# uci-cbcl/esm-efficient

Hardware: AMD Instinct MI355X
Metric: residues/sec ESM2-650M fwd, 50k packed tokens; % bf16 MFMA peak; 1/2/4/8 GPU (higher is better)
Workload: dtype bf16

## Files before the change

### esm-efficient_amd/csrc/attn.hip

```cpp
#include "common.h"
#include "launch.h"
#include "gemm.h"

#include <atomic>
#include <type_traits>

namespace esme {

static constexpr int QT = 128;
static constexpr int KT = 64;
static constexpr int kAttnDma0 = 3, kAttnDma1 = 11;

struct AttnArgs {
    const u16* q; const u16* k; const u16* v; int64_t ld;
    u16* o; int64_t ldo;
    const int32_t* cu;
    int H;
    float scale_log2;
    int nqt;
    int nhb;
    float thr;
    int spec;
    const int32_t* order;
};

template <int D>
__device__ __forceinline__ int kswz(int row) {
    constexpr int CPR = D / 8;
    constexpr int RPB = 16 / CPR;
    return (row / RPB) & (CPR - 1);
}

template <int D, int QB, bool F16 = false>
__global__ __launch_bounds__(256, 2) void attn_varlen_kernel(const AttnArgs a) {
    constexpr int DS = D / 16;
    constexpr int DB = (D + 31) / 32;
    constexpr int CPR = D / 8;
    constexpr int KCH = KT * CPR;
    constexpr int KI = (KCH + 255) / 256;
    constexpr int DQ = D / 4;
    constexpr int DQ_HI_BITS = (D == 16 ? 0 : D == 32 ? 1 : D == 64 ? 2 : 3);
    constexpr int VI = (16 * DQ + 255) / 256;
    constexpr int K_BYTES = KT * D * 2;
    constexpr int BUF = K_BYTES + D * 128;
    const float THR = a.thr;

    __shared__ __attribute__((aligned(16))) char smem[2 * BUF];

    const int tid = threadIdx.x, lane = tid & 63, wave = tid >> 6;
    const int l31 = lane & 31, hi = lane >> 5;
    const int b = a.order ? a.order[blockIdx.z] : (int)blockIdx.z, h = blockIdx.y;
    const int s0 = a.cu[b], S = a.cu[b + 1] - s0;
    const int q0 = blockIdx.x * (QT * QB);
    if (q0 >= S) return;

    const unsigned int ld = (unsigned int)a.ld;
    const u16* qb = a.q + (int64_t)s0 * a.ld + h * D;
    const u16* kb = a.k + (int64_t)s0 * a.ld + h * D;
    const u16* vb = a.v + (int64_t)s0 * a.ld + h * D;

    int qrow[QB];
    bool blk_active[QB];
    bf16x8 qf[QB][DS];
#pragma unroll
    for (int b = 0; b < QB; ++b) {
        const int r0 = q0 + (wave * QB + b) * 32;
        qrow[b] = r0 + l31;
        blk_active[b] = r0 < S;
        const unsigned int qc = qrow[b] < S ? qrow[b] : S - 1;
#pragma unroll
        for (int ds = 0; ds < DS; ++ds)
            qf[b][ds] = *reinterpret_cast<const bf16x8*>(qb + (qc * ld + ds * 16 + hi * 8));
    }
    const bool wave_active = blk_active[0];

    unsigned int koff[KI];
    int krow[KI];
#pragma unroll
    for (int i = 0; i < KI; ++i) {
        const int c = i * 256 + tid;
        krow[i] = c / CPR;
        koff[i] = (unsigned int)(c % CPR) * 8u;
    }
    int v_dq[VI], v_kq[VI];
#pragma unroll
    for (int i = 0; i < VI; ++i) {
        const int rest = (lane >> 4) | (wave << 2) | (i << 4);
        v_dq[i] = (lane & 3) | ((rest & ((1 << DQ_HI_BITS) - 1)) << 2);
        v_kq[i] = ((lane >> 2) & 3) | ((rest >> DQ_HI_BITS) << 2);
    }
    u32x4 kreg[KI];
    u32x2 vreg[VI][4];
    auto load_tile = [&](int kv0) {
        const bool full = kv0 + KT <= S;
#pragma unroll
        for (int i = 0; i < KI; ++i) {
            if (KCH >= 256 * KI || krow[i] < KT) {
                unsigned int row = kv0 + krow[i];
                if (!full) row = row < (unsigned int)S ? row : S - 1;
                kreg[i] = *reinterpret_cast<const u32x4*>(kb + (row * ld + koff[i]));
            }
        }
#pragma unroll
        for (int i = 0; i < VI; ++i) {
            if (v_kq[i] < 16) {
#pragma unroll
// ... 388 lines not shown
#pragma unroll
                        for (int j = 0; j < 8; ++j) p[j] -= ph[j];
                        pf[NPT - 1][kbk][s] = __builtin_bit_cast(bf16x8, pack8t<F16>(p));
                    }
                }
            l_run += psum;

            const char* Vt = buf + 2 * K_BYTES;
#pragma unroll
            for (int i = 0; i < DB; ++i) {
                int drow = i * 32 + l31;
                if (D < 32) drow &= (D - 1);
                const char* rp = Vt + drow * 128;
                const int sw = (drow >> 1) & 7;
#pragma unroll
                for (int kbk = 0; kbk < 2; ++kbk)
#pragma unroll
                    for (int s = 0; s < 2; ++s) {
                        const bf16x8 vh = *reinterpret_cast<const bf16x8*>(rp + (((kbk * 4 + s * 2 + hi) ^ sw) << 4));
                        if constexpr (!QKP) {
                            ESME_LDS_CHECK(rp + V_BYTES + (((kbk * 4 + s * 2 + hi) ^ sw) << 4), 16, smem, 2 * BUF);
                            const bf16x8 vl = *reinterpret_cast<const bf16x8*>(rp + V_BYTES + (((kbk * 4 + s * 2 + hi) ^ sw) << 4));
                            oacc[i] = mfma_32x32x16<F16>(vl, pf[0][kbk][s], oacc[i]);
                            oacc[i] = mfma_32x32x16<F16>(vh, pf[NPT - 1][kbk][s], oacc[i]);
                        }
                        oacc[i] = mfma_32x32x16<F16>(vh, pf[0][kbk][s], oacc[i]);
                    }
            }
        }
        if (t + 1 < ntiles) {
            store_tile(smem + ((t + 1) & 1) * BUF);
            if (t + 2 < ntiles) load_tile(kv0 + 2 * KT);
        }
        __syncthreads();
    }

    if (!wave_active) return;
    const float l_tot = l_run + __shfl_xor(l_run, 32, 64);
    const float inv = 1.0f / l_tot;
    if (qrow < S) {
        u16* op = a.o + (int64_t)(s0 + qrow) * a.ldo + h * D;
#pragma unroll
        for (int i = 0; i < DB; ++i)
#pragma unroll
            for (int g = 0; g < 4; ++g) {
                const int d = i * 32 + 8 * g + 4 * hi;
                if (d < D) {
                    float o4[4];
#pragma unroll
                    for (int e = 0; e < 4; ++e) o4[e] = oacc[i][4 * g + e] * inv;
                    const u32x2 pk = {pack16<F16>(o4[0], o4[1]), pack16<F16>(o4[2], o4[3])};
                    *reinterpret_cast<u32x2*>(op + d) = pk;
                    if constexpr (!QKP) {
                        const u32x2 pl = {pack16<F16>(o4[0] - lo16<F16>(pk[0]), o4[1] - hi16<F16>(pk[0])), pack16<F16>(o4[2] - lo16<F16>(pk[1]), o4[3] - hi16<F16>(pk[1]))};
                        *reinterpret_cast<u32x2*>(op + sa.lo_out + d) = pl;
                    }
                }
            }
    }
}


template <int NW, bool QP = false, int D = 64, bool F16 = false>
__global__ __launch_bounds__(NW * 64, 2) void attn_pp64_kernel(const AttnArgs a) {
    constexpr float S0 = (QP && F16) ? -4.0f : 0.0f;
    constexpr int DS = D / 16, DB = D / 32, NT = NW * 64;
    constexpr int ROWB = D * 2;
    constexpr int K_BYTES = KT * D * 2;
    constexpr int SLOT = K_BYTES + D * 128;
    constexpr int ROWS = NW * 64;
    constexpr int NPV = 4 * DB, NQK = 2 * DS, NM = NPV + NQK;
    constexpr int PPS = 16 / NM;
    static_assert(D == 64 || D == 32, "head dims 64 and 32");
    static_assert(NW == 4 || (NW == 8 && D == 64), "4 waves (8: head dim 64 only)");
    extern __shared__ __attribute__((aligned(16))) char smem[];

    const int tid = threadIdx.x, lane = tid & 63;
    const int wave = __builtin_amdgcn_readfirstlane(tid >> 6);
    const int l31 = lane & 31, hi = lane >> 5;
    const unsigned int xcd = blockIdx.x & 7u, bi = blockIdx.x >> 3;
    const int qt = (int)(bi % (unsigned int)a.nqt);
    const unsigned int hb = (bi / (unsigned int)a.nqt) * 8u + xcd;
    if (hb >= (unsigned int)a.nhb) return;
    const int h = (int)(hb % (unsigned int)a.H), bi_seq = (int)(hb / (unsigned int)a.H);
    const int b = a.order ? a.order[bi_seq] : bi_seq;
    const int s0 = a.cu[b], S = a.cu[b + 1] - s0;
    const int q0 = qt * ROWS;
    if (q0 >= S) return;

    const unsigned int ld = (unsigned int)a.ld;
    const u16* qb = a.q + (int64_t)s0 * a.ld + h * D;
    const unsigned int kv_bytes = ((unsigned int)(S - 1) * ld + D) * 2u;
    auto make_rsrc = [&](const u16* p) -> u32x4 {
        const uint64_t v = (uint64_t)(uintptr_t)p;
        return u32x4{(unsigned int)__builtin_amdgcn_readfirstlane((int)(unsigned int)v),
                     (unsigned int)__builtin_amdgcn_readfirstlane((int)((unsigned int)(v >> 32) & 0xffffu)),
                     (unsigned int)__builtin_amdgcn_readfirstlane((int)kv_bytes), 0x00020000u};
    };
    const u32x4 krs = make_rsrc(a.k + (int64_t)s0 * a.ld + h * D);
    const u32x4 vrs = make_rsrc(a.v + (int64_t)s0 * a.ld + h * D);
    auto dma16 = [&](const u32x4 rs, const unsigned int voff, const char* dst) {
        ESME_LDS_CHECK(dst, 1024, smem, 4 * SLOT);
        const unsigned int d = (unsigned int)__builtin_amdgcn_readfirstlane((int)(unsigned int)(uintptr_t)dst);
        unsigned int keep;
        asm volatile("s_mov_b32 %0, m0\n\ts_mov_b32 m0, %2\n\ts_nop 0\n\tbuffer_load_dwordx4 %1, %3, 0 offen lds\n\ts_mov_b32 m0, %0"
                     : "=&s"(keep) : "v"(voff), "s"(d), "s"(rs) : "memory");
    };

    bf16x8 qf[2][DS];
    const int wrow0 = q0 + wave * 64;
    const bool wave_active = wrow0 < S;
#pragma unroll
    for (int bb = 0; bb < 2; ++bb) {
        const int qr = wrow0 + bb * 32 + l31;
        const unsigned int qc = qr < S ? qr : S - 1;
#pragma unroll
        for (int ds = 0; ds < DS; ++ds)
            qf[bb][ds] = *reinterpret_cast<const bf16x8*>(qb + (qc * ld + ds * 16 + hi * 8));
    }

    constexpr int KI = K_BYTES / (NW * 1024);
    constexpr int CPR = D / 8;
    const unsigned int tile_bytes = (unsigned int)KT * ld * 2u;
    unsigned int kg0, vg0;
    {
        const int r = wave * (64 / CPR) + lane / CPR, pch = lane % CPR;
        kg0 = ((unsigned int)r * ld + ((pch ^ kswz<D>(r)) * 8)) * 2u;
        vg0 = ((unsigned int)r * ld + ((D == 64 ? (pch ^ (((r >> 1) & 1) << 2)) : pch) * 8)) * 2u;
    }
    const unsigned int kg_step = (unsigned int)(NW * (64 / CPR)) * ld * 2u;
    auto dma_k = [&](int tile, char* slot) {
        const unsigned int base = (unsigned int)tile * tile_bytes + kg0;
#pragma unroll
        for (int i = 0; i < KI; ++i)
            dma16(krs, base + i * kg_step, slot + (i * NW + wave) * 1024);
    };
    auto dma_v = [&](int tile, char* slot) {
        const unsigned int base = (unsigned int)tile * tile_bytes + vg0;
#pragma unroll
        for (int i = 0; i < KI; ++i)
            dma16(vrs, base + i * kg_step, slot + K_BYTES + (i * NW + wave) * 1024);
    };

    const int krow_perm = (l31 & 3) | (((l31 >> 3) & 1) << 2) | (((l31 >> 2) & 1) << 3) | (l31 & 16);
    int kfo[DS];
#pragma unroll
    for (int i = 0; i < DS; ++i) kfo[i] = krow_perm * ROWB + (((i * 2 + hi) ^ kswz<D>(krow_perm)) << 4);
    int vb[DB];
    {
        const int j = (lane & 15) >> 2, p = lane & 3, gsel = (lane >> 4) & 1;
#pragma unroll
        for (int db = 0; db < DB; ++db) vb[db] = K_BYTES + (hi * 8 + j) * ROWB + (D == 64 ? ((db ^ (j >> 1)) * 64) : 0) + gsel * 32 + p * 8;
    }
    typedef short s16x4 __attribute__((ext_vector_type(4)));
    auto vfrag = [&](const char* Vs, const int db, const int ks) -> bf16x8 {
        typedef __attribute__((address_space(3))) s16x4* ltr_t;
        const char* p = Vs + vb[db] + ks * (16 * ROWB);
        ESME_LDS_CHECK(p, 8, smem, 4 * SLOT); ESME_LDS_CHECK(p + 4 * ROWB, 8, smem, 4 * SLOT);
        const s16x4 lo = __builtin_amdgcn_ds_read_tr16_b64_v4i16((ltr_t)(p));
        const s16x4 up = __builtin_amdgcn_ds_read_tr16_b64_v4i16((ltr_t)(p + 4 * ROWB));
        return __builtin_bit_cast(bf16x8, __builtin_shufflevector(lo, up, 0, 1, 2, 3, 4, 5, 6, 7));
    };

    f32x16 oacc[2][DB], sacc[2][2];
    u32x4 pw[2][2][2];
    float mc[2], lrun[2];
    const float c = a.scale_log2, thr = a.thr;
// ... 634 lines not shown
    static std::atomic<unsigned long long> done{0ull};
    if (const int rc = raise_dynamic_lds(done, kern, smem, "attn")) return rc;
    sa.a.nqt = (max_len + 127) / 128;
    const int64_t blocks = (int64_t)sa.a.nqt * (((int64_t)sa.a.H * B + 7) / 8) * 8;
    if (blocks > 0x7fffffffLL) return fail(ESME_ERR_UNSUPPORTED, "attn: grid too large");
    hipLaunchKernelGGL(kern, dim3((unsigned int)blocks), dim3(256), smem, s, sa);
    return check_launch("attn_varlen_fwd");
}

static constexpr int kMaxGridZ = 65535;

static int generic_launch_ok(int64_t ld_qkv, int max_len, int rows, int B, const int32_t* seq_order, const char* what) {
    if (((int64_t)max_len + rows) * ld_qkv >= (1LL << 32)) {
        snprintf(error_buffer(), kErrorBufferSize, "%s: (max_len + %d) * ld_qkv must stay below 2^32 elements (32-bit row offsets "
                 "inside one sequence)", what, rows);
        return ESME_ERR_UNSUPPORTED;
    }
    if (seq_order && B > kMaxGridZ) {
        snprintf(error_buffer(), kErrorBufferSize, "%s: seq_order is not supported with more than 65535 sequences", what);
        return ESME_ERR_ARG;
    }
    return ESME_OK;
}

static AttnArgs sequence_chunk(AttnArgs a, int b0, int nb) {
    a.cu += b0;
    a.nhb = a.H * nb;
    return a;
}

template <int D, int QB, bool F16>
static int launch_generic(const AttnArgs& a, int B, int max_len, hipStream_t s) {
    constexpr int rows = QT * QB;
    if (const int rc = generic_launch_ok(a.ld, max_len, rows, B, a.order, "attn")) return rc;
    return for_sequence_chunks(B, kMaxGridZ, [&](int b0, int nb) {
        const dim3 grid((unsigned int)((max_len + rows - 1) / rows), (unsigned int)a.H, (unsigned int)nb);
        hipLaunchKernelGGL((attn_varlen_kernel<D, QB, F16>), grid, dim3(256), 0, s, sequence_chunk(a, b0, nb));
        return check_launch("attn_varlen_fwd");
    });
}

template <int D, bool F16, bool QKP>
static int launch_split(const AttnSplitArgs& sa, int B, int max_len, const char* what, hipStream_t s) {
    constexpr int smem = 2 * (2 * KT * D * 2 + (QKP ? 1 : 2) * D * 128);
    if (const int rc = generic_launch_ok(sa.a.ld, max_len, QT, B, sa.a.order, what)) return rc;
    auto kern = attn_split_kernel<D, F16, QKP>;
    if (smem >= 64 * 1024) {
        static std::atomic<unsigned long long> done{0ull};
        if (const int rc = raise_dynamic_lds(done, kern, smem, "attn_split")) return rc;
    }
    return for_sequence_chunks(B, kMaxGridZ, [&](int b0, int nb) {
        const dim3 grid((unsigned int)((max_len + QT - 1) / QT), (unsigned int)sa.a.H, (unsigned int)nb);
        hipLaunchKernelGGL(kern, grid, dim3(256), smem, s, AttnSplitArgs{sequence_chunk(sa.a, b0, nb), sa.lo_in, sa.lo_out});
        return check_launch("attn_varlen_fwd_split");
    });
}

static int attn_entry_checks(const char* pre, const void* q, const void* k, const void* v, const void* o, const int32_t* cu_lens, int B,
                             int64_t T, int H, int d, int max_len, bool strides_ok, const char* strides_what, bool* empty) {
    auto bad = [&](const char* what) {
        snprintf(error_buffer(), kErrorBufferSize, "%s: %s", pre, what);
        return ESME_ERR_ARG;
    };
    *empty = false;
    if (!(B >= 0 && T >= 0 && H > 0 && d > 0 && max_len >= 0)) return bad("bad sizes");
    if (T == 0 || B == 0) { *empty = true; return ESME_OK; }
    if (!(q && k && v && o && cu_lens)) return bad("null pointer");
    if (!strides_ok) return bad(strides_what);
    if (!(aligned16(q) && aligned16(k) && aligned16(v) && (reinterpret_cast<uintptr_t>(o) & 7u) == 0)) return bad("misaligned");
    if (!(max_len > 0 && H <= 65535)) return bad("max_len must be > 0, H <= 65535");
    return ESME_OK;
}

static AttnArgs attn_args(const void* q, const void* k, const void* v, int64_t ld_qkv, void* o, int64_t ld_o, const int32_t* cu_lens, int B, int H,
                          float scale_log2, const int32_t* seq_order) {
    return AttnArgs{(const u16*)q, (const u16*)k, (const u16*)v, ld_qkv, (u16*)o, ld_o, cu_lens, H, scale_log2, 1, H * B, 0.0f, 0, seq_order};
}
static constexpr float kLog2e = 1.4426950408889634f;

static bool pipelined_ok(int d, const void* o, int64_t ld_o, int64_t ld_qkv, int max_len) {
    return (d == 64 || d == 32) && ld_o % 8 == 0 && aligned16(o) && ((int64_t)max_len + KT) * ld_qkv * 2 < 0xffffffffLL;
}

static int attn_fwd(const void* q, const void* k, const void* v, int64_t ld_qkv, void* o, int64_t ld_o, const int32_t* cu_lens,
                    int B, int64_t T, int H, int d, int max_len, float softmax_scale, void* stream, bool exact,
                    const esme_attn_opts_t* opts) {
    ESME_CHECK_ARG(!opts || opts->struct_bytes == (int)sizeof(esme_attn_opts_t), "attn: options struct of another ABI");
    const int variant = opts ? opts->variant : 0;
    const int force_qb = opts ? opts->q_blocks : 0;
    bool empty;
    if (const int rc = attn_entry_checks("attn", q, k, v, o, cu_lens, B, T, H, d, max_len,
                                         ld_qkv % 8 == 0 && ld_qkv >= (int64_t)H * d && ld_o % 4 == 0 && ld_o >= (int64_t)H * d,
                                         "bad row strides", &empty); rc || empty) return rc;
    const bool f16 = opts && opts->f16;
    const bool qp = opts && opts->q_prescaled;
    ESME_CHECK_ARG(!(f16 && qp) || ((d == 64 || d == 32) && ld_o % 8 == 0 && aligned16(o)),
                   "attn: fp16 operands combine with q_prescaled for head dims 64 / 32 only (the ping-pong kernel's fixed-reference form; "
                   "variants 1 / 2, and strides for which (max_len + 64) rows pass 2^32 bytes, run the generic kernel with a unit scale)");
    AttnArgs a = attn_args(q, k, v, ld_qkv, o, ld_o, cu_lens, B, H, qp ? 1.0f : softmax_scale * kLog2e, opts ? opts->seq_order : nullptr);
    if (!exact) { a.thr = opts ? opts->defer_max_thr : 8.0f; a.spec = opts ? opts->speculative : 1; }
    const hipStream_t s = (hipStream_t)stream;
    const char* const bad_dim = "attn: head dim must be 16, 32, 64 or 128";
    const bool pipelined = pipelined_ok(d, o, ld_o, ld_qkv, max_len) && !(f16 && qp && (variant == 1 || variant == 2));
    if (pipelined && variant == 2)
        return dispatch_head_dim<64, 32>(d, bad_dim, [&](auto D) {
            return dispatch_flags([&](auto F16, auto QP) { return launch_sb<D(), F16(), false, QP() && !F16()>(AttnSplitArgs{a, 0, 0}, B, max_len, s); }, f16, qp);
        });
    if (pipelined && variant != 1) {
        if (variant == 8 && d == 64 && !f16) return launch_pp64<8, false, 64, false>(a, B, max_len, s);
        return dispatch_head_dim<64, 32>(d, bad_dim, [&](auto D) {
            return dispatch_flags([&](auto F16, auto QP) { return launch_pp64<4, QP(), D(), F16()>(a, B, max_len, s); }, f16, qp);
        });
    }
    const bool two = (force_qb ? force_qb : (max_len >= 192 ? 2 : 1)) == 2;
    return dispatch_head_dim<16, 32, 64, 128>(d, bad_dim, [&](auto D) {
        return dispatch_flags([&](auto F16, auto TWO) { return launch_generic<D(), (TWO() && D() <= 64) ? 2 : 1, F16()>(a, B, max_len, s); }, f16, two);
    });
}

extern "C" int esme_hip_attn_varlen_fwd_split(const void* q, const void* k, const void* v, int64_t ld_qkv, int64_t lo_qkv, void* o,
                                              int64_t ld_o, int64_t lo_o, const int32_t* cu_lens, int B, int64_t T, int H, int d,
                                              int max_len, float softmax_scale, const int32_t* seq_order, void* stream) {
    bool empty;
    if (const int rc = attn_entry_checks("attn_split", q, k, v, o, cu_lens, B, T, H, d, max_len,
                                         ld_qkv % 8 == 0 && lo_qkv % 8 == 0 && lo_qkv > 0 && ld_o % 4 == 0 && lo_o % 4 == 0 &&
                                             lo_o >= (int64_t)H * d && ld_o >= lo_o + (int64_t)H * d,
                                         "bad row strides / pair offsets", &empty); rc || empty) return rc;
    const AttnSplitArgs sa{attn_args(q, k, v, ld_qkv, o, ld_o, cu_lens, B, H, softmax_scale * kLog2e, seq_order), lo_qkv, lo_o};
    return dispatch_head_dim<16, 32, 64, 128>(d, "attn_split: head dim must be 16, 32, 64 or 128", [&](auto D) {
        return launch_split<D(), false, false>(sa, B, max_len, "attn_split", (hipStream_t)stream);
    });
}

extern "C" int esme_hip_attn_varlen_fwd_qkpair_f16_opts(const void* q, const void* k, const void* v, int64_t ld_qkv, int64_t lo_qk, void* o,
                                                        int64_t ld_o, const int32_t* cu_lens, int B, int64_t T, int H, int d,
                                                        int max_len, float softmax_scale, const esme_attn_opts_t* opts, void* stream) {
    ESME_CHECK_ARG(!opts || opts->struct_bytes == (int)sizeof(esme_attn_opts_t), "attn_qkpair: options struct of another ABI");
    bool empty;
    if (const int rc = attn_entry_checks("attn_qkpair", q, k, v, o, cu_lens, B, T, H, d, max_len,
                                         ld_qkv % 8 == 0 && lo_qk % 8 == 0 && lo_qk > 0 && ld_o % 4 == 0 && ld_o >= (int64_t)H * d,
                                         "bad row strides / pair offset", &empty); rc || empty) return rc;
    const AttnSplitArgs sa{attn_args(q, k, v, ld_qkv, o, ld_o, cu_lens, B, H, softmax_scale * kLog2e, opts ? opts->seq_order : nullptr), lo_qk, 0};
    const hipStream_t s = (hipStream_t)stream;
    const char* const bad_dim = "attn_qkpair: head dim must be 16, 32 or 64";
    if (opts && opts->variant == 2 && pipelined_ok(d, o, ld_o, ld_qkv, max_len))
        return dispatch_head_dim<64, 32>(d, bad_dim, [&](auto D) { return launch_sb<D(), true, true, false>(sa, B, max_len, s); });
    return dispatch_head_dim<16, 32, 64>(d, bad_dim, [&](auto D) {
        return launch_split<D(), true, true>(sa, B, max_len, "attn_qkpair", s);
    });
}

extern "C" int esme_hip_attn_varlen_fwd_qkpair_f16(const void* q, const void* k, const void* v, int64_t ld_qkv, int64_t lo_qk, void* o,
                                                   int64_t ld_o, const int32_t* cu_lens, int B, int64_t T, int H, int d,
                                                   int max_len, float softmax_scale, const int32_t* seq_order, void* stream) {
    esme_attn_opts_t o1{(int)sizeof(esme_attn_opts_t), 0, 0, 0.0f, 0, seq_order, 0, 1};
    return esme_hip_attn_varlen_fwd_qkpair_f16_opts(q, k, v, ld_qkv, lo_qk, o, ld_o, cu_lens, B, T, H, d, max_len, softmax_scale, &o1, stream);
}

extern "C" int esme_hip_attn_varlen_fwd(const void* q, const void* k, const void* v, int64_t ld_qkv, void* o,
                                        int64_t ld_o, const int32_t* cu_lens, int B, int64_t T, int H, int d,
                                        int max_len, float softmax_scale, void* stream) {
    return attn_fwd(q, k, v, ld_qkv, o, ld_o, cu_lens, B, T, H, d, max_len, softmax_scale, stream, false, nullptr);
}

extern "C" int esme_hip_attn_varlen_fwd_opts(const void* q, const void* k, const void* v, int64_t ld_qkv, void* o,
                                             int64_t ld_o, const int32_t* cu_lens, int B, int64_t T, int H, int d,
                                             int max_len, float softmax_scale, const esme_attn_opts_t* opts, void* stream) {
    return attn_fwd(q, k, v, ld_qkv, o, ld_o, cu_lens, B, T, H, d, max_len, softmax_scale, stream, false, opts);
}

extern "C" int esme_hip_attn_varlen_fwd_exact(const void* q, const void* k, const void* v, int64_t ld_qkv, void* o,
                                              int64_t ld_o, const int32_t* cu_lens, int B, int64_t T, int H, int d,
                                              int max_len, float softmax_scale, void* stream) {
    return attn_fwd(q, k, v, ld_qkv, o, ld_o, cu_lens, B, T, H, d, max_len, softmax_scale, stream, true, nullptr);
}
```

### esm-efficient_amd/csrc/gemm.h

```cpp
#pragma once
#include "common.h"
#include "launch.h"

namespace esme {

struct GemmArgs {
    const u16* A = nullptr; int64_t lda = 0;
    const u16* W = nullptr;
    const u16* bias = nullptr;
    const u16* resid = nullptr; int64_t ldr = 0;
    u16* C = nullptr; int64_t ldc = 0;
    int64_t M = 0; int N = 0; int K = 0;
    float alpha = 0.f;
    int tiles_n = 0;
    int vec_ok = 0;
    const u16* cosT = nullptr; const u16* sinT = nullptr; const int32_t* pos = nullptr; int max_len = 0; int rot_cols = 0;
    int tiles_m = 0, gm = 1, gn = 1;
    int nt_store = 0;
    int stagger = 0;
    const float* ln_partial = nullptr; int ln_nblk = 0; int ln_dim = 0; float ln_eps = 0.f; const float* ln_c1 = nullptr; const float* ln_c2 = nullptr;
    float* stats_out = nullptr;
    int64_t stat_ld = 0;
    unsigned long long* trace = nullptr;
    int opt_gm = 0, opt_gn = 0, opt_persist = -1;
    float q_scale = 0.f; int q_cols = 0;
    float* resid32 = nullptr; int64_t ld32 = 0;
    int kt_wrap = 0; int64_t pair_off = 0; float* c32 = nullptr; int64_t ldc32 = 0;
    int f16 = 0;
    const float* ps_in = nullptr; const float* ps_out = nullptr;
    const int32_t* ext_sel = nullptr; int ext_n = 0; int64_t ext_off = 0;
    int ext_base = 0;
    int* ovf = nullptr;
    int pair_cols = 0;
    unsigned int* col_absmax = nullptr;
    unsigned int* qk_sumsq = nullptr;
    int stream_out = 0;
};

#ifdef ESME_GEMM_TRACE
#define ESME_TUNE_STORE_OK (a.nt_store != 2)
#else
#define ESME_TUNE_STORE_OK true
#endif

#ifdef ESME_GEMM_TRACE
#define ESME_TRACE_STRIDE 32
#define ESME_TRACE_MARK(i) do { if (a.trace && threadIdx.x == 0) a.trace[(size_t)blockIdx.x * ESME_TRACE_STRIDE + (i)] = __builtin_readcyclecounter(); } while (0)
#define ESME_TRACE_REAL(i) do { if (a.trace && threadIdx.x == 0) a.trace[(size_t)blockIdx.x * ESME_TRACE_STRIDE + (i)] = __builtin_amdgcn_s_memrealtime(); } while (0)
#define ESME_TRACE_SEAM(i, t) do { if (a.trace && threadIdx.x == 0 && trace_tile == (t)) a.trace[(size_t)blockIdx.x * ESME_TRACE_STRIDE + (i)] = __builtin_readcyclecounter(); } while (0)
#else
#define ESME_TRACE_MARK(i) do {} while (0)
#define ESME_TRACE_REAL(i) do {} while (0)
#define ESME_TRACE_SEAM(i, t) do {} while (0)
#endif

static constexpr int BK = 64;
constexpr bool WTN_OK(int bn, int wn) { return bn / wn == 64; }

typedef __attribute__((address_space(1))) const void* gptr_t;
typedef __attribute__((address_space(3))) void* lptr_t;


}
```

### esm-efficient_amd/csrc/gemm.hip

```cpp
#include "gemm.h"
#include <atomic>
#include <cstdlib>

namespace esme {

static constexpr int kGemmP3N = 4;
static constexpr int kNtMinMB = 256;

template <int BM, int BN, int WM, int WN, int EPI, int ROTD = 0, bool LNF = false, bool STATS = false, bool PERSIST = false, bool R32 = false, bool PAIR = false, bool F16 = false, bool RP = false>
__global__ __launch_bounds__(WM * WN * 64) void gemm_bf16_kernel(const GemmArgs a) {
    static_assert(!RP || (F16 && EPI == ESME_EPI_RESIDUAL && !R32 && !PAIR && !LNF && ROTD == 0), "pair stream: fp16 residual epilogue");
    static_assert(!F16 || ((!PAIR || (LNF && EPI == ESME_EPI_NONE)) && (EPI != ESME_EPI_RESIDUAL || R32 || RP)),
                  "fp16 operands: plain / GELU / SwiGLU epilogues, the fp32- / pair-stream residual epilogues, pair output of the LN-folded plain epilogue");
    static_assert(!LNF || EPI != ESME_EPI_RESIDUAL, "LN fold applies to the consumers of a LayerNorm");
    static_assert(!R32 || EPI == ESME_EPI_RESIDUAL, "the fp32 residual stream belongs to the residual epilogue");
    static_assert(!PAIR || (EPI != ESME_EPI_RESIDUAL && (!LNF || F16) && !STATS && !PERSIST), "(hi, lo) pair output: plain / GELU / SwiGLU epilogues of the split-operand mode; fp16: the LN-folded plain epilogue");
    static_assert(!STATS || (EPI == ESME_EPI_RESIDUAL && WTN_OK(BN, WN) && BN / WN == 64 && (WN == 2 || WN == 4)), "row statistics are emitted by the residual epilogue");
    static_assert(ROTD == 0 || (EPI == ESME_EPI_NONE && (ROTD == 16 || ROTD == 32 || ROTD == 64) && WTN_OK(BN, WN)),
                  "fused rotary: plain epilogue, head dim 16/32/64, 64-column wave tiles");
    constexpr int NW = WM * WN;
    constexpr int NT = NW * 64;
    constexpr int WTM = BM / WM, WTN = BN / WN;
    constexpr int FM = WTM / 16, FN = WTN / 16;
    constexpr int FMH = FM / 2;
    static_assert(FM % 2 == 0, "wave tile rows split in two halves");
    constexpr int A_ROWS_BYTES = BM * 128, W_ROWS_BYTES = BN * 128;
    constexpr int STAGE = A_ROWS_BYTES + W_ROWS_BYTES;
    constexpr int IA = BM * 8 / NT, IW = BN * 8 / NT;
    static_assert(BM * 8 % NT == 0 && BN * 8 % NT == 0, "tile/threads mismatch");
    static_assert(EPI != ESME_EPI_SWIGLU || WTN == 64, "swiglu needs 64-wide wave tiles");

    extern __shared__ __attribute__((aligned(16))) char smem[];
    constexpr int LDS_BYTES = 2 * (BM + BN) * 128 + ((LNF || ROTD > 0) ? BM * 12 + BN * 8 : 0) + (STATS ? WN * BM * 8 : 0) + (RP ? 2 * BN * 8 : 0);
    (void)LDS_BYTES;

    const int tid = threadIdx.x;
    const int lane = tid & 63;
    const int wave = __builtin_amdgcn_readfirstlane(tid >> 6);
    constexpr bool P8 = (NW == 8 && WM == 2 && WN == 4 && BM == 256 && BN == 256);
    const int wm = P8 ? (wave >> 2) : wave % WM, wn = P8 ? (wave & 3) : wave / WM;
    const int l15 = lane & 15, lq = lane >> 4;
    ESME_TRACE_REAL(8);
    ESME_TRACE_MARK(0);

#ifdef ESME_GEMM_TRACE
    if (a.stagger > 0 && blockIdx.x < 256) {
        const int n = (blockIdx.x * a.stagger) >> 8;
        for (int i = 0; i < n; ++i) __builtin_amdgcn_s_sleep(16);
    }
#endif
    unsigned int pid, pid_end = 0u, pid_step = 0u;
    if constexpr (PERSIST) {
        const unsigned int nblk = (unsigned int)(a.tiles_m * a.tiles_n);
        const unsigned int q = nblk >> 3, r = nblk & 7u, xcd = blockIdx.x & 7u, slot = blockIdx.x >> 3;
        const unsigned int base = (xcd < r) ? xcd * (q + 1) : r * (q + 1) + (xcd - r) * q;
        pid_step = gridDim.x >> 3;
        pid = base + slot;
        pid_end = base + q + (xcd < r ? 1u : 0u);
        if (pid >= pid_end) return;
    } else {
        pid = xcd_remap(blockIdx.x, gridDim.x);
    }
    int64_t m0;
    int n0;
    auto tile_coords = [&](const unsigned int id) {
        const int per_band = a.gm * a.tiles_n;
        const int band = id / per_band, lb = id - band * per_band;
        const int rows = min(a.gm, a.tiles_m - band * a.gm);
        const int grp = rows * a.gn;
        const int ng = lb / grp, rg = lb - ng * grp;
        const int tile_n = ng * a.gn + rg / rows;
        const int64_t tile_m = (int64_t)band * a.gm + rg % rows;
        m0 = tile_m * BM;
        n0 = tile_n * BN;
    };
    tile_coords(pid);

    const u16* srcA[IA];
    const u16* srcW[IW];
    auto set_sources = [&]() {
        int ln = lane;
        if constexpr (PERSIST) asm volatile("" : "+v"(ln));
#pragma unroll
        for (int i = 0; i < IA; ++i) {
            const int q = (i * NW + wave) * 64 + ln;
            const int row = q >> 3, c = (q & 7) ^ ((row >> 1) & 7);
            const int trow = P8 ? ((row >> 6) & 1) * WTM + (row >> 7) * (WTM / 2) + (row & 63) : row;
            int64_t gr = m0 + trow;
            gr = gr < a.M ? gr : a.M - 1;
            srcA[i] = a.A + gr * a.lda + c * 8;
        }
#pragma unroll
        for (int i = 0; i < IW; ++i) {
            const int q = (i * NW + wave) * 64 + ln;
            const int row = q >> 3, c = (q & 7) ^ ((row >> 1) & 7);
            const int tcol = P8 ? ((row >> 5) & 3) * WTN + (row >> 7) * (WTN / 2) + (row & 31) : row;
            int gr = n0 + tcol;
            gr = gr < a.N ? gr : a.N - 1;
            srcW[i] = a.W + (int64_t)gr * (a.kt_wrap > 0 ? a.kt_wrap * BK : a.K) + c * 8;
        }
    };
    set_sources();

    auto w_k0 = [&](const int kt) { return ((a.kt_wrap > 0 && kt >= a.kt_wrap) ? kt - a.kt_wrap : kt) * BK; };
    auto stage = [&](int kt, int buf) {
        char* base = smem + buf * STAGE;
        const int k0 = kt * BK, k0w = w_k0(kt);
#pragma unroll
        for (int i = 0; i < IA; ++i)
            __builtin_amdgcn_global_load_lds((gptr_t)(srcA[i] + k0), (lptr_t)(base + (i * NW + wave) * 1024), 16, 0, 0);
#pragma unroll
        for (int i = 0; i < IW; ++i)
            __builtin_amdgcn_global_load_lds((gptr_t)(srcW[i] + k0w),
                                             (lptr_t)(base + A_ROWS_BYTES + (i * NW + wave) * 1024), 16, 0, 0);
    };

    const int swz = (l15 >> 1) & 7;
    int coff[2];
#pragma unroll
    for (int ks = 0; ks < 2; ++ks) coff[ks] = ((ks * 4 + lq) ^ swz) << 4;
    const int rowA = (P8 ? wm * (WTM / 2) + l15 : wm * WTM + l15) * 128;
    const int rowW = A_ROWS_BYTES + (P8 ? wn * (WTN / 2) + l15 : wn * WTN + l15) * 128;

    f32x4 acc[FN][FM];
#pragma unroll
    for (int i = 0; i < FN; ++i)
#pragma unroll
        for (int j = 0; j < FM; ++j)
#pragma unroll
            for (int r = 0; r < 4; ++r) acc[i][j][r] = 0.f;

    const int KT = a.K / BK;
    struct FragW { bf16x8 v[FN]; };
    struct FragA { bf16x8 v[FMH]; };
    auto rdW = [&](FragW& f, const char* base, int ks) {
#pragma unroll
        for (int i = 0; i < FN; ++i) f.v[i] = *reinterpret_cast<const bf16x8*>(base + rowW + i * 16 * 128 + coff[ks]);
    };
    auto rdA = [&](FragA& f, const char* base, int ks, int h) {
#pragma unroll
        for (int j = 0; j < FMH; ++j) f.v[j] = *reinterpret_cast<const bf16x8*>(base + rowA + (h * FMH + j) * 16 * 128 + coff[ks]);
    };
    static_assert(IA % 2 == 0 && IW % 2 == 0, "the LDS-DMA pieces of a K-tile split in two halves");
    constexpr int NP = IA + IW;
    auto stage_piece = [&](int kt, int buf, int p) {
        char* base = smem + buf * STAGE;
        const int k0 = kt * BK;
        ESME_LDS_CHECK(p < IA ? base + (p * NW + wave) * 1024 : base + A_ROWS_BYTES + ((p - IA) * NW + wave) * 1024, 1024, smem, 2 * STAGE);
// ... 783 lines not shown
        for (int i = 0; i < FN; ++i)
#pragma unroll
            for (int j = 0; j < FM; ++j)
#pragma unroll
                for (int r = 0; r < 4; ++r) acc[i][j][r] = 0.f;
        asm volatile("s_waitcnt lgkmcnt(0)" ::: "memory");
        ESME_TRACE_SEAM(26, 1);
        __builtin_amdgcn_s_barrier();
    }
    }
}

static int persist_default() {
    static const int v = [] { const char* e = getenv("ESME_GEMM_PERSIST"); return e ? (atoi(e) != 0) : 1; }();
    return v;
}
static int cu_count() {
    static std::atomic<int> cached[64];
    int dev = 0;
    (void)hipGetDevice(&dev);
    int v = cached[dev & 63].load(std::memory_order_relaxed);
    if (v <= 0) {
        if (hipDeviceGetAttribute(&v, hipDeviceAttributeMultiprocessorCount, dev) != hipSuccess || v <= 0) v = 256;
        cached[dev & 63].store(v, std::memory_order_relaxed);
    }
    return v;
}

struct GemmForm {
    int epi, rotd;
    bool lnf, stats, r32, pair, f16, rp;
    constexpr unsigned key() const { return epi | rotd << 2 | lnf << 9 | stats << 10 | r32 << 11 | pair << 12 | f16 << 13 | rp << 14; }
};

#define ESME_GEMM_FORMS(X)                                                                                                                                      \
                                                                      \
    X(ESME_EPI_NONE, 0, 0, 0, 0, 1, 0, 0) X(ESME_EPI_NONE, 16, 0, 0, 0, 1, 0, 0) X(ESME_EPI_NONE, 32, 0, 0, 0, 1, 0, 0) X(ESME_EPI_NONE, 64, 0, 0, 0, 1, 0, 0)  \
    X(ESME_EPI_GELU, 0, 0, 0, 0, 1, 0, 0) X(ESME_EPI_SWIGLU, 0, 0, 0, 0, 1, 0, 0)                                                                               \
                                                      \
    X(ESME_EPI_NONE, 0, 1, 0, 0, 1, 1, 0) X(ESME_EPI_NONE, 16, 1, 0, 0, 1, 1, 0) X(ESME_EPI_NONE, 32, 1, 0, 0, 1, 1, 0) X(ESME_EPI_NONE, 64, 1, 0, 0, 1, 1, 0)  \
                                                                             \
    X(ESME_EPI_NONE, 0, 1, 0, 0, 0, 1, 0) X(ESME_EPI_NONE, 0, 0, 0, 0, 0, 1, 0) X(ESME_EPI_NONE, 16, 1, 0, 0, 0, 1, 0) X(ESME_EPI_NONE, 32, 1, 0, 0, 0, 1, 0)   \
    X(ESME_EPI_NONE, 64, 1, 0, 0, 0, 1, 0) X(ESME_EPI_GELU, 0, 1, 0, 0, 0, 1, 0) X(ESME_EPI_GELU, 0, 0, 0, 0, 0, 1, 0) X(ESME_EPI_SWIGLU, 0, 1, 0, 0, 0, 1, 0)   \
    X(ESME_EPI_RESIDUAL, 0, 0, 1, 0, 0, 1, 1) X(ESME_EPI_RESIDUAL, 0, 0, 0, 0, 0, 1, 1) X(ESME_EPI_RESIDUAL, 0, 0, 1, 1, 0, 1, 0) X(ESME_EPI_RESIDUAL, 0, 0, 0, 1, 0, 1, 0) \
                 \
    X(ESME_EPI_NONE, 0, 1, 0, 0, 0, 0, 0) X(ESME_EPI_NONE, 0, 0, 0, 0, 0, 0, 0) X(ESME_EPI_NONE, 16, 1, 0, 0, 0, 0, 0) X(ESME_EPI_NONE, 16, 0, 0, 0, 0, 0, 0)   \
    X(ESME_EPI_NONE, 32, 1, 0, 0, 0, 0, 0) X(ESME_EPI_NONE, 32, 0, 0, 0, 0, 0, 0) X(ESME_EPI_NONE, 64, 1, 0, 0, 0, 0, 0) X(ESME_EPI_NONE, 64, 0, 0, 0, 0, 0, 0) \
    X(ESME_EPI_GELU, 0, 1, 0, 0, 0, 0, 0) X(ESME_EPI_GELU, 0, 0, 0, 0, 0, 0, 0) X(ESME_EPI_SWIGLU, 0, 1, 0, 0, 0, 0, 0) X(ESME_EPI_SWIGLU, 0, 0, 0, 0, 0, 0, 0) \
    X(ESME_EPI_RESIDUAL, 0, 0, 1, 1, 0, 0, 0) X(ESME_EPI_RESIDUAL, 0, 0, 0, 1, 0, 0, 0) X(ESME_EPI_RESIDUAL, 0, 0, 1, 0, 0, 0, 0) X(ESME_EPI_RESIDUAL, 0, 0, 0, 0, 0, 0, 0)

constexpr bool has_persistent_twin(int bm, int bn, int rotd, bool pair, bool rp) { return bm == 256 && bn == 256 && rotd == 0 && !pair && !rp; }

static int gemm_form(GemmForm& f, const GemmArgs& a, int epi, int rotd, bool lnf, bool stats) {
    if (epi < ESME_EPI_NONE || epi > ESME_EPI_SWIGLU) return fail(ESME_ERR_ARG, "gemm: unknown epilogue");
    const bool plain = epi == ESME_EPI_NONE, resid = epi == ESME_EPI_RESIDUAL, f16 = a.f16 != 0, has_pair = a.pair_off != 0;
    if (plain && rotd != 0 && rotd != 16 && rotd != 32 && rotd != 64) return fail(ESME_ERR_UNSUPPORTED, "gemm: fused rotary needs head dim 16, 32 or 64");
    if (has_pair && !f16 && resid) return fail(ESME_ERR_ARG, "gemm: pair output does not combine with the residual epilogue");
    f.epi = epi; f.rotd = plain ? rotd : 0; f.f16 = f16;
    f.rp = f16 && has_pair && resid;
    f.pair = has_pair && (f16 ? plain : !resid);
    f.r32 = resid && !f.rp && (f16 || a.resid32);
    f.stats = resid && stats;
    f.lnf = !resid && (f.pair ? f16 : lnf);
    if (f16 && !f.lnf && f.rotd) return fail(ESME_ERR_UNSUPPORTED, "gemm: fp16 fused rotary runs LayerNorm-folded only");
    if (f16 && !f.lnf && epi == ESME_EPI_SWIGLU) return fail(ESME_ERR_UNSUPPORTED, "gemm: fp16 SwiGLU runs LayerNorm-folded only");
    return ESME_OK;
}

template <int BM, int BN>
static void set_raster(GemmArgs& a) {
    a.tiles_n = (a.N + BN - 1) / BN;
    a.tiles_m = (int)((a.M + BM - 1) / BM);
    const double w_bytes = 2.0 * a.N * a.K;
    if (a.opt_gm > 0) { a.gm = a.opt_gm; a.gn = a.opt_gn > 0 ? a.opt_gn : a.tiles_n; }
    else if (w_bytes <= 3.5e6 || a.tiles_n <= 6) { a.gm = 1; a.gn = a.tiles_n; }
    else if (a.tiles_n % 5 == 0) { a.gm = 6; a.gn = 5; }
    else { a.gm = 8; a.gn = 4; }
    if (a.gn > a.tiles_n) a.gn = a.tiles_n;
    if (a.gm > a.tiles_m) a.gm = a.tiles_m;
    if (a.gm < 1) a.gm = 1;
    if (a.gn < 1) a.gn = 1;
}

template <int BM, int BN, int WM, int WN, int EPI, int ROTD, bool LNF, bool STATS, bool R32, bool PAIR, bool F16, bool RP, bool PERSIST = false>
static int launch_one(GemmArgs& a, hipStream_t s) {
    constexpr int smem = 2 * (BM + BN) * 128 + ((LNF || ROTD > 0) ? BM * 12 + BN * 8 : 0) + (STATS ? WN * BM * 8 : 0) + (RP ? 2 * BN * 8 : 0);
    set_raster<BM, BN>(a);
    int64_t blocks = (int64_t)a.tiles_m * a.tiles_n;
    if (blocks > 0x7fffffffLL) return fail(ESME_ERR_UNSUPPORTED, "gemm: grid too large");
    if constexpr (!PERSIST && has_persistent_twin(BM, BN, ROTD, PAIR, RP)) {
        const int ncu = cu_count() & ~7;
        const bool want = a.opt_persist < 0 ? persist_default() != 0 : a.opt_persist != 0;
        if (want && a.vec_ok && ncu >= 8 && blocks >= 2 * (int64_t)ncu) return launch_one<BM, BN, WM, WN, EPI, ROTD, LNF, STATS, R32, PAIR, F16, RP, true>(a, s);
    }
    if constexpr (PERSIST) blocks = cu_count() & ~7;
    auto kern = gemm_bf16_kernel<BM, BN, WM, WN, EPI, ROTD, LNF, STATS, PERSIST, R32, PAIR, F16, RP>;
    if (smem >= 64 * 1024) {
        static std::atomic<unsigned long long> done{0ull};
        if (const int rc = raise_dynamic_lds(done, kern, smem, "gemm")) return rc;
    }
    hipLaunchKernelGGL(kern, dim3((unsigned int)blocks), dim3(WM * WN * 64), smem, s, a);
    return check_launch("gemm_bf16");
}

template <int BM, int BN, int WM, int WN>
static int launch_gemm(GemmArgs& a, const GemmForm& f, hipStream_t s) {
    switch (f.key()) {
#define ESME_GEMM_CASE(E, R, L, S, R32, P, H, RP) \
        case GemmForm{E, R, L, S, R32, P, H, RP}.key(): return launch_one<BM, BN, WM, WN, E, R, L, S, R32, P, H, RP>(a, s);
        ESME_GEMM_FORMS(ESME_GEMM_CASE)
#undef ESME_GEMM_CASE
        default: return fail(ESME_ERR_UNSUPPORTED, "gemm: this combination of epilogue and fusions is not built");
    }
}

}

using namespace esme;

#ifdef ESME_GEMM_TRACE
static int g_nt_store = 0, g_stagger = 0;
extern "C" void esme_hip_debug_set_gemm_nt(int v) { g_nt_store = v; }
extern "C" void esme_hip_debug_set_gemm_stagger(int v) { g_stagger = v; }
static unsigned long long* g_trace = nullptr;
extern "C" void esme_hip_debug_set_gemm_trace(void* p) { g_trace = (unsigned long long*)p; }
#endif

static int pick_tile(int64_t M, int N, const esme_gemm_opts_t* opts) {
    if (opts && opts->tile) return opts->tile;
    const int64_t big_tiles = ((M + 255) / 256) * ((N + 255) / 256);
    return (N >= 256 && big_tiles >= 160) ? 2 : 1;
}

extern "C" int esme_hip_gemm_stats_blocks_opts(int64_t M, int N, const esme_gemm_opts_t* opts) {
    const int bn = pick_tile(M, N, opts) == 2 ? 256 : 128;
    return (N + bn - 1) / bn;
}
extern "C" int esme_hip_gemm_stats_blocks(int64_t M, int N) { return esme_hip_gemm_stats_blocks_opts(M, N, nullptr); }

static bool column_split_pays(const GemmArgs& a, const GemmForm& f, const esme_gemm_opts_t* opts) {
    if (!f.rp || (opts && opts->tile) || a.N <= 256 || a.N % 256 != 128) return false;
    const int64_t tm = (a.M + 255) / 256, ncu = cu_count() & ~7;
    const int64_t full = tm * ((a.N + 255) / 256), main_tiles = tm * (a.N / 256);
    return ncu >= 8 && main_tiles >= 160 && (main_tiles + ncu - 1) / ncu < (full + ncu - 1) / ncu;
}

static GemmArgs last_columns(const GemmArgs& a, int c0) {
    GemmArgs t = a;
    t.N = 128;
    t.W = a.W + (int64_t)c0 * (a.kt_wrap > 0 ? a.kt_wrap * BK : a.K);
    t.C = a.C + c0;
    if (a.bias) t.bias = a.bias + c0;
    if (a.resid) t.resid = a.resid + c0;
    if (a.resid32) t.resid32 = a.resid32 + c0;
    if (a.ps_in) t.ps_in = a.ps_in + c0;
    if (a.ps_out) t.ps_out = a.ps_out + c0;
    if (a.col_absmax) t.col_absmax = a.col_absmax + c0;
    if (a.stats_out) t.stats_out = a.stats_out + 2 * (int64_t)(c0 / 256) * a.stat_ld;
    if (a.ext_off) { t.ext_base = c0; t.ext_off = a.ext_off - c0; }
    return t;
}

enum GemmMode { kBf16, kSplitOperand, kF16, kF16PairOut, kF16PairStream };

extern "C" int esme_hip_gemm_bf16_opts(const void* A, int64_t lda, const void* W, const void* bias, const void* resid,
                                       int64_t ldr, void* C, int64_t ldc, int64_t M, int N, int K, int epilogue,
                                       float alpha, const esme_gemm_fusion_t* fu, const esme_gemm_opts_t* opts, void* stream) {
    auto aligned = [](const void* p, unsigned bytes) { return (reinterpret_cast<uintptr_t>(p) & (bytes - 1)) == 0; };
    ESME_CHECK_ARG(!opts || (opts->struct_bytes == (int)sizeof(esme_gemm_opts_t) && opts->tile >= 0 && opts->tile <= 2),
                   "gemm: options struct of another ABI or bad tile");
    ESME_CHECK_ARG(M >= 0 && N > 0 && K > 0, "gemm: bad sizes");
    ESME_CHECK_ARG(epilogue >= ESME_EPI_NONE && epilogue <= ESME_EPI_SWIGLU, "gemm: unknown epilogue");
    if (M == 0) return ESME_OK;
    ESME_CHECK_ARG(A && W && C, "gemm: null pointer");
    if (K % BK != 0) ESME_FAIL(ESME_ERR_UNSUPPORTED, "gemm: K must be a multiple of 64");
    const bool plain = epilogue == ESME_EPI_NONE, residual = epilogue == ESME_EPI_RESIDUAL, swiglu = epilogue == ESME_EPI_SWIGLU;
    const int n_out = swiglu ? N / 2 : N;
    if (swiglu && N % 64 != 0) ESME_FAIL(ESME_ERR_UNSUPPORTED, "gemm: swiglu needs N % 64 == 0");
    ESME_CHECK_ARG(lda >= K && lda % 8 == 0 && ldc >= n_out, "gemm: bad lda/ldc");
    ESME_CHECK_ARG(aligned16(A) && aligned16(W), "gemm: A and W must be 16-byte aligned");
    ESME_CHECK_ARG(!bias || aligned(bias, 8), "gemm: misaligned bias");
    bool vec_ok = (ldc % 8 == 0) && aligned16(C) && (n_out % 8 == 0) && N >= 8;
    const bool r32 = fu && fu->resid32;
    if (r32) {
        ESME_CHECK_ARG(residual, "gemm: resid32 belongs to the residual epilogue");
        ESME_CHECK_ARG(fu->ld32 >= N && fu->ld32 % 4 == 0 && aligned16(fu->resid32), "gemm: resid32 needs ld32 >= N, ld32 % 4 == 0, 16-byte alignment");
        if (!vec_ok) ESME_FAIL(ESME_ERR_UNSUPPORTED, "gemm: the fp32 residual stream needs a 16-byte addressable C and N % 8 == 0");
    } else if (residual) {
        ESME_CHECK_ARG(resid && ldr >= N, "gemm: residual epilogue needs resid with ldr >= N");
        vec_ok = vec_ok && (ldr % 8 == 0) && aligned16(resid);
    }
    if (swiglu && !vec_ok) ESME_FAIL(ESME_ERR_UNSUPPORTED, "gemm: swiglu needs ldc % 8 == 0 and a 16-byte aligned C");

    GemmArgs a{};
    a.A = (const u16*)A; a.lda = lda; a.W = (const u16*)W; a.bias = (const u16*)bias; a.resid = (const u16*)resid; a.ldr = ldr;
    a.C = (u16*)C; a.ldc = ldc; a.M = M; a.N = N; a.K = K; a.alpha = alpha; a.vec_ok = vec_ok; a.stat_ld = M;
#ifdef ESME_GEMM_TRACE
    a.nt_store = g_nt_store; a.stagger = g_stagger; a.trace = g_trace;
#endif
    if (opts) { a.opt_gm = opts->raster_gm; a.opt_gn = opts->raster_gn; a.opt_persist = opts->persist; }
    if (r32) { a.resid32 = fu->resid32; a.ld32 = fu->ld32; }
    int rotd = 0;
    bool lnf = false, stats = false;
    if (fu) {
        const GemmMode mode = fu->f16 && fu->pair_off ? (plain ? kF16PairOut : kF16PairStream)
                              : (fu->w_k || fu->pair_off || fu->c32) ? kSplitOperand : fu->f16 ? kF16 : kBf16;
        ESME_CHECK_ARG((!fu->pair_scale_in && !fu->pair_scale_out && !fu->ext_off) || (mode == kF16PairStream && residual),
                       "gemm: pair_scale_in / pair_scale_out / ext_* belong to the fp16 pair stream's residual epilogue");
        ESME_CHECK_ARG(!fu->pair_cols || mode == kF16PairOut, "gemm: pair_cols belongs to the fp16 pair output");
        ESME_CHECK_ARG(!fu->col_absmax || (mode == kF16PairStream && residual), "gemm: col_absmax belongs to the fp16 pair stream's residual epilogue");
        ESME_CHECK_ARG(!fu->qk_sumsq || (fu->f16 && fu->ln_partial && fu->head_dim != 0 && !fu->pair_off), "gemm: qk_sumsq belongs to the fp16 LN-folded projection with fused rotary (single output)");
        switch (mode) {
            case kF16PairOut:
                ESME_CHECK_ARG(fu->ln_partial && !r32 && !fu->w_k && !fu->c32 && !fu->stats_out, "gemm: the fp16 pair output belongs to the LN-folded plain epilogue");
                ESME_CHECK_ARG(fu->pair_off >= N && fu->pair_off % 8 == 0 && ldc >= fu->pair_off + (fu->pair_cols > 0 ? fu->pair_cols : N) && fu->pair_cols >= 0 && fu->pair_cols % 256 == 0,
// ... 117 lines not shown
```

Baseline: 800,500.

## Reverse tile walk in residual GEMM and attention to reuse producer's cached output

Adds a reverse-order tile traversal flag to the residual-epilogue GEMM (for K > N shapes whose input exceeds a size threshold) and to the pipelined attention kernel (for equal-length batches whose QKV exceeds 256 MB). The consumer kernel then starts on the rows the previous kernel wrote last, which are most likely still resident in the last-level cache, instead of the oldest rows that have likely been evicted. It adds a small index remap per tile and debug overrides for forcing the walk. The attention path only triggers when every sequence has max_len, so packed variable-length batches may not use it.

```diff
diff --git a/esm-efficient_amd/csrc/attn.hip b/esm-efficient_amd/csrc/attn.hip
--- a/esm-efficient_amd/csrc/attn.hip
+++ b/esm-efficient_amd/csrc/attn.hip
@@ -22,6 +22,7 @@
     float thr;
     int spec;
     const int32_t* order;
+    int rev;
 };
 
 template <int D>
@@ -576,7 +577,8 @@
     const int qt = (int)(bi % (unsigned int)a.nqt);
     const unsigned int hb = (bi / (unsigned int)a.nqt) * 8u + xcd;
     if (hb >= (unsigned int)a.nhb) return;
-    const int h = (int)(hb % (unsigned int)a.H), bi_seq = (int)(hb / (unsigned int)a.H);
+    const unsigned int hbw = a.rev ? (unsigned int)a.nhb - 1u - hb : hb;
+    const int h = (int)(hbw % (unsigned int)a.H), bi_seq = (int)(hbw / (unsigned int)a.H);
     const int b = a.order ? a.order[bi_seq] : bi_seq;
     const int s0 = a.cu[b], S = a.cu[b + 1] - s0;
     const int q0 = qt * ROWS;
@@ -1377,6 +1379,16 @@
     return (d == 64 || d == 32) && ld_o % 8 == 0 && aligned16(o) && ((int64_t)max_len + KT) * ld_qkv * 2 < 0xffffffffLL;
 }
 
+static constexpr double kCacheBytes = 256.0 * 1048576.0;
+static std::atomic<int> g_attn_walk{-1};
+static int attn_walk_reverse(int B, int64_t T, int max_len, int64_t ld_qkv) {
+    if (T != (int64_t)B * max_len) return 0;
+    const int forced = g_attn_walk.load(std::memory_order_relaxed);
+    if (forced >= 0) return forced != 0;
+    return (double)T * (double)ld_qkv * 2.0 > kCacheBytes;
+}
+extern "C" void esme_hip_debug_set_attn_walk(int v) { g_attn_walk.store(v < 0 ? -1 : (v != 0), std::memory_order_relaxed); }
+
 static int attn_fwd(const void* q, const void* k, const void* v, int64_t ld_qkv, void* o, int64_t ld_o, const int32_t* cu_lens,
                     int B, int64_t T, int H, int d, int max_len, float softmax_scale, void* stream, bool exact,
                     const esme_attn_opts_t* opts) {
@@ -1402,6 +1414,7 @@
             return dispatch_flags([&](auto F16, auto QP) { return launch_sb<D(), F16(), false, QP() && !F16()>(AttnSplitArgs{a, 0, 0}, B, max_len, s); }, f16, qp);
         });
     if (pipelined && variant != 1) {
+        a.rev = attn_walk_reverse(B, T, max_len, ld_qkv);
         if (variant == 8 && d == 64 && !f16) return launch_pp64<8, false, 64, false>(a, B, max_len, s);
         return dispatch_head_dim<64, 32>(d, bad_dim, [&](auto D) {
             return dispatch_flags([&](auto F16, auto QP) { return launch_pp64<4, QP(), D(), F16()>(a, B, max_len, s); }, f16, qp);
diff --git a/esm-efficient_amd/csrc/gemm.h b/esm-efficient_amd/csrc/gemm.h
--- a/esm-efficient_amd/csrc/gemm.h
+++ b/esm-efficient_amd/csrc/gemm.h
@@ -35,6 +35,7 @@
     unsigned int* col_absmax = nullptr;
     unsigned int* qk_sumsq = nullptr;
     int stream_out = 0;
+    int rev = 0;
 };
 
 #ifdef ESME_GEMM_TRACE
diff --git a/esm-efficient_amd/csrc/gemm.hip b/esm-efficient_amd/csrc/gemm.hip
--- a/esm-efficient_amd/csrc/gemm.hip
+++ b/esm-efficient_amd/csrc/gemm.hip
@@ -63,7 +63,12 @@
     }
     int64_t m0;
     int n0;
-    auto tile_coords = [&](const unsigned int id) {
+    constexpr bool WALK_REV = EPI == ESME_EPI_RESIDUAL && !R32 && !RP && !F16;
+    auto tile_coords = [&](unsigned int id) {
+        if constexpr (WALK_REV) {
+            const unsigned int m = 0u - (unsigned int)a.rev;
+            id = (id ^ m) + (m & (unsigned int)(a.tiles_m * a.tiles_n));
+        }
         const int per_band = a.gm * a.tiles_n;
         const int band = id / per_band, lb = id - band * per_band;
         const int rows = min(a.gm, a.tiles_m - band * a.gm);
@@ -1013,10 +1018,20 @@
     if (a.gn < 1) a.gn = 1;
 }
 
+static std::atomic<int> g_walk{-1};
+template <int EPI, bool R32, bool F16, bool RP>
+static int walk_reverse(const GemmArgs& a) {
+    if (EPI != ESME_EPI_RESIDUAL || R32 || F16 || RP) return 0;
+    const int forced = g_walk.load(std::memory_order_relaxed);
+    if (forced >= 0) return forced != 0;
+    return a.K > a.N && (double)a.M * a.K * 2.0 > kNtMinMB * 1048576.0;
+}
+
 template <int BM, int BN, int WM, int WN, int EPI, int ROTD, bool LNF, bool STATS, bool R32, bool PAIR, bool F16, bool RP, bool PERSIST = false>
 static int launch_one(GemmArgs& a, hipStream_t s) {
     constexpr int smem = 2 * (BM + BN) * 128 + ((LNF || ROTD > 0) ? BM * 12 + BN * 8 : 0) + (STATS ? WN * BM * 8 : 0) + (RP ? 2 * BN * 8 : 0);
     set_raster<BM, BN>(a);
+    a.rev = walk_reverse<EPI, R32, F16, RP>(a);
     int64_t blocks = (int64_t)a.tiles_m * a.tiles_n;
     if (blocks > 0x7fffffffLL) return fail(ESME_ERR_UNSUPPORTED, "gemm: grid too large");
     if constexpr (!PERSIST && has_persistent_twin(BM, BN, ROTD, PAIR, RP)) {
@@ -1062,6 +1077,8 @@
     const int64_t big_tiles = ((M + 255) / 256) * ((N + 255) / 256);
     return (N >= 256 && big_tiles >= 160) ? 2 : 1;
 }
+
+extern "C" void esme_hip_debug_set_gemm_walk(int v) { g_walk.store(v < 0 ? -1 : (v != 0), std::memory_order_relaxed); }
 
 extern "C" int esme_hip_gemm_stats_blocks_opts(int64_t M, int N, const esme_gemm_opts_t* opts) {
     const int bn = pick_tile(M, N, opts) == 2 ? 256 : 128;
```

Measured after the change: 803,100 (median of 6 runs). About the same (+0.3%).
